# AzureLeon1/DiffSpectra

Hardware: AMD Instinct MI355X
Metric: molecules/sec, 1000-step QM9S all-spectra sampling (partial run) (higher is better)
Workload: dtype f32 (GEMMs as split-fp16 x3 MFMA with fp32 accumulate; fp32-level accuracy, parity gates unchanged)

## Files before the change

__graft_entry__.py:

```python
from __future__ import annotations

import os
import subprocess
import sys

ROOT = os.path.dirname(os.path.abspath(__file__))
if ROOT not in sys.path:
    sys.path.insert(0, ROOT)

CSRC = os.path.join(ROOT, "diffspectra_amd", "csrc")
HIP_SOURCES = [os.path.join(CSRC, n) for n in ("ds_forward.hip", "ds_gemm.hip", "ds_sampler.hip", "ds_spec.hip", "ds_aux.hip", "ds_match.hip", "ds_graph.hip", "ds_mces.hip", "ds_morgan.hip", "ds_subgeom.hip", "ds_mmd.hip", "ds_sets.hip", "ds_valence.hip", "ds_groups.hip", "ds_scaffold.hip", "ds_smiles.hip", "ds_substructure.hip", "ds_stereo.hip", "ds_brics.hip", "ds_mobile.hip", "ds_key.hip", "ds_fraggle.hip", "ds_bestrmsd.hip", "ds_reader.hip", "ds_train.hip", "ds_train_gemm.hip", "ds_train_attn.hip", "ds_train_chain.hip")]
HIP_DEPS = [os.path.join(CSRC, "ds_device.h"), os.path.join(CSRC, "ds_host.h"), os.path.join(CSRC, "ds_train_common.h"), os.path.join(CSRC, "ds_svd3.h"), os.path.join(CSRC, "ds_records.h"), os.path.join(CSRC, "ds_bonds.h"), os.path.join(CSRC, "ds_refine.h"), os.path.join(CSRC, "ds_perceive.h"), os.path.join(CSRC, "ds_mobile.h"), os.path.join(CSRC, "ds_vec.h"), os.path.join(CSRC, "ds_sites.h"),
            os.path.join(ROOT, "include", "diffspectra_hip.h"), os.path.join(ROOT, "include", "diffspectra_train.h"),
            os.path.join(ROOT, "include", "diffspectra_sets.h"), os.path.join(ROOT, "include", "diffspectra_valence.h"), os.path.join(ROOT, "include", "diffspectra_groups.h"),
            os.path.join(ROOT, "include", "diffspectra_scaffold.h"), os.path.join(ROOT, "include", "diffspectra_smiles.h"), os.path.join(ROOT, "include", "diffspectra_substructure.h"), os.path.join(ROOT, "include", "diffspectra_stereo.h"), os.path.join(ROOT, "include", "diffspectra_brics.h"), os.path.join(ROOT, "include", "diffspectra_mobile.h"), os.path.join(ROOT, "include", "diffspectra_key.h"), os.path.join(ROOT, "include", "diffspectra_fraggle.h"), os.path.join(ROOT, "include", "diffspectra_rmsd.h"), os.path.join(ROOT, "include", "diffspectra_reader.h"),
            os.path.join(ROOT, "include", "diffspectra_tiles.h"), os.path.join(ROOT, "include", "diffspectra_step.h"), os.path.join(ROOT, "include", "diffspectra_solver.h")]
LIB = os.path.join(ROOT, "diffspectra_amd", "libdiffspectra_hip.so")
OBJ_DIR = os.path.join(ROOT, "build", "obj")
BASE_FLAGS = ["--offload-arch=gfx950", "-O3", "-std=c++17", "-fPIC", "-Wno-pass-failed", "-Wno-unused-value"]
OPT_FLAGS = ["-mllvm", "-amdgpu-mfma-vgpr-form=1"]
LIBRARY_STATE = "not built"


def _digest(paths):
    import hashlib
    h = hashlib.sha1()
    for p in paths:
        h.update(os.path.basename(p).encode() + b"\0")
        with open(p, "rb") as f:
            h.update(f.read())
    return h.hexdigest()


def _read(path):
    try:
        with open(path) as f:
            return f.read()
    except OSError:
        return None


def _stale(target, deps):
    return not os.path.exists(target) or any(not os.path.exists(d) for d in deps) or _read(target + ".src") != _digest(deps)


def _compile(hipcc, src, obj, flags):
    cmd = [hipcc, *flags, "-c", src, "-o", obj]
    print("[build]", " ".join(cmd), file=sys.stderr, flush=True)
    r = subprocess.run(cmd, cwd=ROOT, capture_output=True, text=True)
# ... 83 lines not shown
```

diffspectra_amd/abi.py:

```python
from __future__ import annotations

import ctypes as C
import os
import re
import struct as _struct
from typing import Dict, List, NamedTuple, Tuple

_INCLUDE = os.path.join(os.path.dirname(os.path.dirname(os.path.abspath(__file__))), "include")

_FIELD_CODES = {"int64_t": "q", "int32_t": "i", "uint32_t": "I", "uint64_t": "Q", "float": "f"}
_CTYPES = {"P": C.c_void_p, "q": C.c_int64, "i": C.c_int32, "I": C.c_uint32, "Q": C.c_uint64, "f": C.c_float}
_ARG_CTYPES = {"*": C.c_void_p, "int": C.c_int, "int32_t": C.c_int32, "int64_t": C.c_int64, "uint32_t": C.c_uint32, "uint64_t": C.c_uint64,
               "float": C.c_float, "double": C.c_double}


class Prototype(NamedTuple):
    name: str
    ret: str
    params: List[Tuple[str, str]]

    @property
    def argtypes(self):
        return [_ARG_CTYPES[t] for _, t in self.params]

# ... 65 lines not shown
        return [name for name in self.prototypes if name.startswith(prefix)]

    def bind(self, lib: C.CDLL) -> None:
        for p in self.prototypes.values():
            fn = getattr(lib, p.name)
            fn.restype = None if p.ret == "void" else C.c_int
            fn.argtypes = p.argtypes

    def packer(self, name: str) -> _struct.Struct:
        return _struct.Struct("@" + "".join(code for _, code in self.structs[name]))

    def ctypes_struct(self, name: str):
        def ctype(code):
            return _CTYPES[code[-1]] * int(code[:-1]) if len(code) > 1 else _CTYPES[code]
        return type(name, (C.Structure,), {"_fields_": [(f_, ctype(code)) for f_, code in self.structs[name]]})


SAMPLING = Header("diffspectra_hip.h")
TRAINING = Header("diffspectra_train.h")
SETS = Header("diffspectra_sets.h")
VALENCE = Header("diffspectra_valence.h")
GROUPS = Header("diffspectra_groups.h")
SCAFFOLD = Header("diffspectra_scaffold.h")
SMILES = Header("diffspectra_smiles.h")
SUBSTRUCTURE = Header("diffspectra_substructure.h")
STEREO = Header("diffspectra_stereo.h")
BRICS = Header("diffspectra_brics.h")
MOBILE = Header("diffspectra_mobile.h")
KEY = Header("diffspectra_key.h")
FRAGGLE = Header("diffspectra_fraggle.h")
RMSD = Header("diffspectra_rmsd.h")
READER = Header("diffspectra_reader.h")
TILES = Header("diffspectra_tiles.h")
STEP = Header("diffspectra_step.h")
SOLVER = Header("diffspectra_solver.h")
```

diffspectra_amd/csrc/ds_forward.hip:

```cpp
#include <hip/hip_runtime.h>
#include <math.h>
#include <stdint.h>
#include <stdlib.h>

#include <atomic>
#include <mutex>
#include <utility>
#include <vector>

#include "../../include/diffspectra_hip.h"
#include "../../include/diffspectra_step.h"
#include "../../include/diffspectra_tiles.h"
#include "ds_device.h"
#include "ds_host.h"

#define ADAC DS_ADA_COLS
constexpr int DS_NODE_PF = 8;
constexpr int DS_NODE_PF2 = 4;
constexpr int DS_QKV_PF = 4;
constexpr int DS_QKV_PF_WIDE = 4;
constexpr int DS_NODE_TILE64_MIN_PER_CU = 4;
constexpr int DS_TWO_STREAM_MAX_PAIRS = 400000;

#ifdef DS_STAMPS
#define DS_STAMP_INIT()                                                                                 \
  unsigned long long _sa[16] = {0, 0, 0, 0, 0, 0, 0, 0, 0, 0, 0, 0, 0, 0, 0, 0};                        \
  unsigned long long _t0 = __builtin_amdgcn_s_memtime()
#define DS_STAMP(i)                                                                                     \
  do {                                                                                                  \
    const unsigned long long _t1 = __builtin_amdgcn_s_memtime();                                        \
    _sa[i] += _t1 - _t0;                                                                                \
    _t0 = _t1;                                                                                          \
  } while (0)
#define DS_STAMP_W(i)                                                                                   \
  do {                                                                                                  \
    asm volatile("s_waitcnt vmcnt(0) lgkmcnt(0)" ::: "memory");                                         \
    DS_STAMP(i);                                                                                        \
  } while (0)
#define DS_STAMP_FLUSH(t)                                                                               \
  do {                                                                                                  \
    if (threadIdx.x == (t))                                                                             \
      for (int _i = 0; _i < 16; ++_i)                                                                   \
        if (_sa[_i]) atomicAdd(reinterpret_cast<unsigned long long*>(c.ws.flags + 16) + _i, _sa[_i]);   \
  } while (0)
#else
#define DS_STAMP_INIT()
#define DS_STAMP(i)
#define DS_STAMP_W(i)
#define DS_STAMP_FLUSH(t)
#endif

namespace {

using dst::clear;
using dst::record;
using dst::wait;

struct Ctx {
  ds_layout L;
  ds_workspace ws;
  const float* wbase;
  const int64_t* woff;
  float edge_th, cutoff;
};

__device__ __forceinline__ const float* BW(const Ctx& c, int blk, int slot) {
  return c.wbase + c.woff[blk * DS_W_BLOCK_SLOTS + slot];
}
__device__ __forceinline__ const float* GW(const Ctx& c, int slot) {
  return c.wbase + c.woff[DS_NBLOCKS * DS_W_BLOCK_SLOTS + slot];
}

__device__ __forceinline__ float rbf_feature(float x, int k, const float* __restrict__ mean, const float* __restrict__ stdv,
                                             const float* __restrict__ astd) {
  if (k == 0) return x;
  const float z = (x - mean[k - 1]) / stdv[k - 1];
  return expf(-0.5f * (z * z)) / astd[k - 1];
}

__global__ void k_time_feat(Ctx c, const float* __restrict__ noise_level, int rows) {
  const int b = blockIdx.x * blockDim.x + threadIdx.x;
  if (b >= rows) return;
  const float* w = GW(c, DS_GW_SIN_W);
  const float x = noise_level[b];
  float* f = c.ws.tfeat + (size_t)b * 24;
  f[0] = x;
  for (int i = 0; i < 8; ++i) {
    const float fr = ((x * w[i]) * 2.0f) * 3.14159265358979323846f;
    f[1 + i] = sinf(fr);
    f[9 + i] = cosf(fr);
  }
  for (int i = 17; i < 24; ++i) f[i] = 0.0f;
}

__global__ void k_pair_flags(Ctx c, const float* __restrict__ cond_x, const float* __restrict__ cond_edge_x) {
  const int p = blockIdx.x * blockDim.x + threadIdx.x;
// ... 245 lines not shown
        }
      }
#pragma unroll
      for (int ps = 0; ps < 2; ++ps) {
        const int row = RW * wv + 8 * half + 4 * ps + g;
        ln_mod_quad256(v[ps], sh[ps], sc[ps]);
#pragma unroll
        for (int u = 0; u < 4; ++u)
          split_store4(&Xh[row][0], 256, 64 * u + 4 * j, row0 + row < c.L.Nn ? v[ps][u] : make_float4(0, 0, 0, 0));
      }
    }
  }
  __syncthreads();
  const float* bias = BW(c, blk, DS_BW_QKV_B) + col0;
  float* qkv = c.ws.qkv + (size_t)row0 * 768 + col0;
  const int valid = c.L.Nn - row0, wave = tid >> 6;
  for (int ch = wave; ch < NCH; ch += NW) {
    asm volatile("" ::: "memory");
    const float b = bias[ch * 32 + (tid & 31)];
    f32x16 acc[2], lo[2];
#pragma unroll
    for (int m = 0; m < 2; ++m)
#pragma unroll
      for (int i = 0; i < 16; ++i) acc[m][i] = b;
    acc_zero<2>(lo);
    wave_mma_h_ring<2, false, 16, PF>(&Xh[0][0], 256, BW(c, blk, DS_BW_QKV_H), 768, 256, col0 + ch * 32, 0, acc, lo);
    split_finish<2>(acc, lo);
    acc_store<2, 768>(acc, qkv + ch * 32, valid, [](int, float v) { return v; });
  }
}
__global__ __launch_bounds__(256) void k_node_qkv(Ctx c, int blk) { node_qkv_tile<4, DS_QKV_PF>(c, blk); }
__global__ __launch_bounds__(512, 2) void k_node_qkv_wide(Ctx c, int blk) { node_qkv_tile<8, DS_QKV_PF_WIDE>(c, blk); }

__global__ __launch_bounds__(1024) void k_attn_fused(Ctx c, int blk) {
  ds_fp16_saturate();
  DS_STAMP_INIT();
  constexpr int NT = 1024, QS = 512 + 32, LDT = 256 + 4, LDY = 2 * 64 + 8, CR = 32, MAXP = DS_MAX_ATOMS * (DS_MAX_ATOMS - 1) / 2;
  __shared__ __attribute__((aligned(16))) float QK[DS_MAX_ATOMS * QS];
  __shared__ __attribute__((aligned(16))) float Tt[2][CR][LDT];
  __shared__ __attribute__((aligned(16))) _Float16 Yc[2][CR][LDY];
  __shared__ __attribute__((aligned(16))) float AL[2][CR][32];
  __shared__ int PT[(MAXP + 15) & ~15];
  __shared__ int VT[32][32];
  static_assert(DS_MAX_ATOMS <= 32 && MAXP <= 511 - CR, "visit table packing");
  static_assert(DS_MAX_ATOMS * 128 <= 4 * NT && DS_MAX_ATOMS * 64 <= 2 * NT && MAXP <= NT, "single-pass staging");
  const int tid = threadIdx.x, wave = tid >> 6, lane = tid & 63, hh = lane >> 5;
  int n0, n, p0, P;
  if (c.L.mol_by_size) {
    const int4 r = reinterpret_cast<const int4*>(c.L.mol_by_size)[blockIdx.x];
    n0 = r.x; n = r.y; p0 = r.z; P = r.w;
  } else {
    const int m = blockIdx.x;
    n0 = c.L.node_off[m]; n = c.L.node_off[m + 1] - n0;
    p0 = c.L.pair_off[m]; P = c.L.pair_off[m + 1] - p0;
  }
  const WStreamH ws_e0 = wstream_h(BW(c, blk, DS_BW_E0_H), 256, 64, (wave & 7) * 32);
  const WStreamH ws_e1 = wstream_h(BW(c, blk, DS_BW_E1_H), 256, 64, (wave & 7) * 32);
  if (n <= 0) return;
  if (P <= 0) {
    for (int i = tid; i < 256; i += NT) c.ws.attn[(size_t)n0 * 256 + i] = 0.0f;
    return;
  }
  const int nch = (P + CR - 1) / CR;
  const bool producer = wave >= 8;
  const int ptid = tid & 511, prow = ptid >> 4, ppiece = ptid & 15;
  const u32x4* ye4 = reinterpret_cast<const u32x4*>(c.ws.ye) + (size_t)p0 * 16;
  auto row_pair = [&](int R) {
    const int d = R / n + 1, i = R - (d - 1) * n;
    int j = i + d;
    if (j >= n) j -= n;
    const int a = min(i, j), b = max(i, j);
    return a * (2 * n - a - 1) / 2 + (b - a - 1);
  };
  auto fetch_y = [&](int ck, bool class_order) {
    const int R = ck * CR + prow;
    const int Rc = min(R, P - 1);
    return ye4[(size_t)(class_order ? PT[Rc] : Rc) * 16 + ppiece];
  };
  auto commit_y = [&](int buf, const u32x4& v) { *reinterpret_cast<u32x4*>(&Yc[buf][prow][ppiece * 8]) = v; };
  h8 wf[2][4];
  auto load_weights = [&](const WStreamH& ws_) {
#pragma unroll
    for (int pl = 0; pl < 2; ++pl)
#pragma unroll
      for (int kb = 0; kb < 4; ++kb) wf[pl][kb] = wload_h(ws_, pl, kb);
  };
  auto project = [&](int buf) {
    f32x16 acc[1], lo[1];
    acc_zero<1>(acc);
    acc_zero<1>(lo);
// ... 50 lines not shown
    }
    f32x4 v[4];
#pragma unroll
    for (int u = 0; u < 4; ++u) {
      const int idx = min(tid + u * NT, n * 128 - 1);
      v[u] = reinterpret_cast<const f32x4*>(c.ws.qkv + (size_t)(n0 + (idx >> 7)) * 768)[idx & 127];
    }
    __builtin_amdgcn_sched_barrier(0);
    auto store_qk = [&]() {
      f32x4* junk = reinterpret_cast<f32x4*>(&Tt[1][0][0]) + tid;
#pragma unroll
      for (int u = 0; u < 4; ++u) {
        const int idx = tid + u * NT;
        f32x4* dst = idx < n * 128 ? reinterpret_cast<f32x4*>(QK) + (idx >> 7) * (QS / 4) + (idx & 127) : junk;
        *dst = v[u];
      }
    };
    if (producer) commit_y(0, y0);
    __syncthreads();
    if (producer) { DS_STAMP(8); } else { DS_STAMP(0); }
    if (producer) {
      produce(y1, y2, false, store_qk);
      load_weights(ws_e1);
    } else {
      store_qk();
      __syncthreads();
      DS_STAMP(1);
      const int row = tid >> 4, hs = tid & 15;
      for (int k = 0; k < nch; ++k) {
        const int pl = k * CR + row;
        if (pl < P) {
          const int e_ = PT[pl];
          float* out = c.ws.lg + (size_t)(p0 + pl) * 32;
          if (hs == 14) {
            const float h0 = (e_ & 0x10000) ? 1.0f : -1e10f, h1 = (e_ & 0x20000) ? 1.0f : -1e10f;
            out[0] = h0; out[1] = h1; out[16] = h0; out[17] = h1;
          } else if (hs < 14) {
            const int a = (e_ >> 8) & 255, b = e_ & 255;
            typedef const volatile f32x2 __attribute__((address_space(3))) * lds_v2;
            lds_v2 t0 = (lds_v2)(&Tt[k & 1][row][hs * 18]);
            lds_v2 qa = (lds_v2)(QK + a * QS + hs * 18);
            lds_v2 qb = (lds_v2)(QK + b * QS + hs * 18);
            lds_v2 ka = (lds_v2)(QK + a * QS + 256 + hs * 18);
            lds_v2 kb = (lds_v2)(QK + b * QS + 256 + hs * 18);
            float s_ab = 0.0f, s_ba = 0.0f;
#pragma unroll
            for (int j0 = 0; j0 < 9; j0 += 3) {
              f32x2 e[3], xa[3], xb[3], ya[3], yb[3];
#pragma unroll
              for (int j = 0; j < 3; ++j) { e[j] = t0[j0 + j]; xa[j] = qa[j0 + j]; xb[j] = qb[j0 + j]; ya[j] = ka[j0 + j]; yb[j] = kb[j0 + j]; }
#pragma unroll
              for (int j = 0; j < 3; ++j) {
                s_ab = __builtin_fmaf(xb[j].x * ya[j].x, e[j].x, s_ab); s_ab = __builtin_fmaf(xb[j].y * ya[j].y, e[j].y, s_ab);
                s_ba = __builtin_fmaf(xa[j].x * yb[j].x, e[j].x, s_ba); s_ba = __builtin_fmaf(xa[j].y * yb[j].y, e[j].y, s_ba);
              }
            }
            out[2 + hs] = s_ab / 4.0f;
            out[16 + 2 + hs] = s_ba / 4.0f;
          }
        }
        DS_STAMP(2);
        __syncthreads();
        DS_STAMP(3);
      }
    }
  }
  __threadfence_block();
  __syncthreads();
  float* V = QK;
  int* ET = reinterpret_cast<int*>(&Tt[0][0][0]);
  {
    const int t = tid >> 5, q = tid & 31, d = (q >> 1) + 1;
    int e = 511;
    if (t < n && q < n - 1) {
      int i, s_;
      if (2 * d == n) {
        i = t < d ? t : t - d;
        s_ = t < d ? t + d : t - d;
      } else {
        int sa = t + d, ib = t - d;
        if (sa >= n) sa -= n;
        if (ib < 0) ib += n;
        const bool first_is_a = t < ib;
        const bool take_a = (q & 1) ? !first_is_a : first_is_a;
        i = take_a ? t : ib;
        s_ = take_a ? sa : ib;
      }
      e = ((d - 1) * n + i) | (s_ << 9) | ((s_ < t ? 0 : 1) << 14);
    }
    VT[t][q] = e;
    const int s = q;
    int eo = -1;
    if (t < n && s < n && s != t) {
      const int lo_ = s < t ? s : t, hi_ = s < t ? t : s;
      eo = (lo_ * (2 * n - lo_ - 1) / 2 + (hi_ - lo_ - 1)) * 32 + (s < t ? 0 : 16);
    }
    ET[t * 32 + s] = eo;
    if (tid < P) PT[tid] = row_pair(tid);
  }
  f32x4 vst[2];
#pragma unroll
  for (int u = 0; u < 2; ++u) {
    const int i0 = min(tid + u * NT, n * 64 - 1);
    vst[u] = reinterpret_cast<const f32x4*>(c.ws.qkv + (size_t)(n0 + (i0 >> 6)) * 768 + 512)[i0 & 63];
  }
  __builtin_amdgcn_sched_barrier(0);
  __syncthreads();
  u32x4 y0 = {0, 0, 0, 0}, y1 = y0, y2 = y0;
  if (producer) {
    y0 = fetch_y(0, true);
    y1 = fetch_y(1, true);
    y2 = fetch_y(2, true);
  }
  auto store_v = [&]() {
    f32x4* junk = reinterpret_cast<f32x4*>(&Yc[0][0][0]) + tid;
#pragma unroll
    for (int u = 0; u < 2; ++u) {
      f32x4* dst = tid + u * NT < n * 64 ? reinterpret_cast<f32x4*>(V) + tid + u * NT : junk;
      *dst = vst[u];
    }
  };
  {
    const int h = lane & 15, sq = (lane >> 4) & 1, t = 2 * wave + hh;
    const int* et = ET + t * 32 + sq;
    float* lgm = c.ws.lg + (size_t)p0 * 32 + h;
    if (t < n) {
      float x[15];
      int eos[15];
      float mx = -INFINITY;
#pragma unroll
      for (int j = 0; j < 15; ++j) eos[j] = et[2 * j];
#pragma unroll
      for (int j = 0; j < 15; ++j) x[j] = lgm[max(eos[j], 0)];
      __builtin_amdgcn_sched_barrier(0);
#pragma unroll
      for (int j = 0; j < 15; ++j) x[j] = eos[j] >= 0 ? x[j] : -INFINITY;
#pragma unroll
      for (int j = 0; j < 15; ++j) mx = fmaxf(mx, x[j]);
      mx = fmaxf(mx, __shfl_xor(mx, 16, 64));
      float sum = 0.0f;
#pragma unroll
      for (int j = 0; j < 15; ++j) {
        x[j] = __expf(x[j] - mx);
        sum += x[j];
      }
      sum += __shfl_xor(sum, 16, 64);
      const float den = sum + 1e-16f;
#pragma unroll
      for (int j = 0; j < 15; ++j)
        if (eos[j] >= 0) lgm[eos[j]] = x[j] / den;
    }
  }
  store_v();
  __threadfence_block();
  __syncthreads();
  if (producer) { DS_STAMP(12); } else { DS_STAMP(4); }
  if (producer) {
    commit_y(0, y0);
    __syncthreads();
    produce(y1, y2, true, [] {});
    DS_STAMP_FLUSH(512);
  } else {
    const int arow = (tid & 255) >> 3, apiece = tid & 7;
    auto fetch_a = [&](int ck) {
      const int R = ck * CR + arow;
      return reinterpret_cast<const u32x4*>(c.ws.lg + (size_t)(p0 + PT[min(R, P - 1)]) * 32)[apiece];
    };
    auto commit_a = [&](int buf, const u32x4& v) {
      if (tid < 256) reinterpret_cast<u32x4*>(&AL[buf][arow][0])[apiece] = v;
    };
    const u32x4 a0 = fetch_a(0);
    u32x4 ab = fetch_a(1), aa = fetch_a(2);
    commit_a(0, a0);
    __syncthreads();
    __syncthreads();
    DS_STAMP(5);
    const int t_me = tid >> 4, q16 = tid & 15;
    const int* vt_row = &VT[t_me][0];
    int vt_q = 0, vt_e = vt_row[0];
    float4 acc[4];
#pragma unroll
    for (int u = 0; u < 4; ++u) acc[u] = make_float4(0, 0, 0, 0);
    auto interval = [&](int k, u32x4& A) {
      if (k + 1 < nch) commit_a((k + 1) & 1, A);
      if (k + 3 < nch) A = fetch_a(k + 3);
      const int R0 = k * CR;
      while ((vt_e & 511) - R0 < CR) {
        const int r = (vt_e & 511) - R0, s_ = (vt_e >> 9) & 31;
        const float4* gp = reinterpret_cast<const float4*>(&Tt[k & 1][r][4 * q16]);
        const float4* vp = reinterpret_cast<const float4*>(V + s_ * 256 + 4 * q16);
        const float* ap = &AL[k & 1][r][((vt_e >> 14) & 1) * 16 + (q16 >> 2)];
        float4 g[4], v[4];
        float al[4];
#pragma unroll
        for (int u = 0; u < 4; ++u) { g[u] = gp[16 * u]; v[u] = vp[16 * u]; al[u] = ap[4 * u]; }
        vt_e = vt_row[++vt_q];
#pragma unroll
        for (int u = 0; u < 4; ++u) {
          acc[u].x += (v[u].x * g[u].x) * al[u]; acc[u].y += (v[u].y * g[u].y) * al[u];
          acc[u].z += (v[u].z * g[u].z) * al[u]; acc[u].w += (v[u].w * g[u].w) * al[u];
        }
      }
      DS_STAMP(6);
      __syncthreads();
      DS_STAMP(7);
    };
    for (int k = 0; k < nch; k += 2) {
      interval(k, ab);
      if (k + 1 >= nch) break;
      interval(k + 1, aa);
    }
    if (t_me < n) {
      float4* o = reinterpret_cast<float4*>(c.ws.attn + (size_t)(n0 + t_me) * 256 + 4 * q16);
#pragma unroll
      for (int u = 0; u < 4; ++u) o[16 * u] = acc[u];
    }
    DS_STAMP_FLUSH(0);
  }
}

__global__ __launch_bounds__(256) void k_node_n2e(Ctx c, int blk) {
  ds_fp16_saturate();
  constexpr int T = 64, LDH = 2 * 256 + 8;
  __shared__ __attribute__((aligned(16))) _Float16 A1[T][LDH];
  const int tid = threadIdx.x, wave = tid >> 6, lane = tid & 63, row0 = blockIdx.x * T;
  const int Nn = c.L.Nn;
  {
    float4 v[16];
#pragma unroll
    for (int u = 0; u < 16; ++u) {
      const int idx = tid + u * 256, row = idx >> 6, k4 = idx & 63;
      v[u] = reinterpret_cast<const float4*>(c.ws.attn + (size_t)min(row0 + row, Nn - 1) * 256)[k4];
    }
#pragma unroll
    for (int u = 0; u < 16; ++u) {
      const int idx = tid + u * 256, row = idx >> 6, k4 = idx & 63;
      split_store4(&A1[row][0], 256, 4 * k4, row0 + row < Nn ? v[u] : make_float4(0, 0, 0, 0));
    }
  }
  __syncthreads();
  const int mt = wave >> 1, cc = wave & 1;
  if (row0 + mt * 32 >= Nn) return;
  f32x16 acc[1], lo[1];
  acc_zero<1>(acc);
// ... 1089 lines not shown
  const int m = blockIdx.x * blockDim.x + threadIdx.x;
  if (m >= c.L.B) return;
  const int n0 = c.L.node_off[m], n = c.L.node_off[m + 1] - n0;
  const bool nan = c.ws.flags[1] != 0;
  float sx = 0.0f, sy = 0.0f, sz = 0.0f;
  for (int a = 0; a < n; ++a) {
    const float* pp = c.ws.pos + (size_t)(n0 + a) * 4;
    if (!nan) { sx += pp[0]; sy += pp[1]; sz += pp[2]; }
  }
  const float fn = (float)n;
  for (int a = 0; a < n; ++a) {
    const float* pp = c.ws.pos + (size_t)(n0 + a) * 4;
    float* o = out_xh + (size_t)c.L.node_dense[n0 + a] * 9;
    const float px = nan ? 0.0f : pp[0], py = nan ? 0.0f : pp[1], pz = nan ? 0.0f : pp[2];
    o[0] = px - sx / fn; o[1] = py - sy / fn; o[2] = pz - sz / fn;
  }
}

__global__ void k_temb_finish(Ctx c, const float* __restrict__ tm3, int tm3_rows, const float* __restrict__ ctx) {
  ds_fp16_saturate();
  const size_t i = (size_t)blockIdx.x * blockDim.x + threadIdx.x;
  if (i >= (size_t)c.L.B * 1024) return;
  const size_t b = i >> 10, col = i & 1023;
  float v = tm3[(tm3_rows == 1 ? 0 : b) * 1024 + col];
  if (ctx) v += ctx[i];
  split_store1(reinterpret_cast<_Float16*>(c.ws.temb_silu) + b * 2048, 1024, (int)col, ds_silu(v));
}

bool make_ctx(Ctx& c, const ds_weights* w, const ds_layout* L, const ds_workspace* ws) {
  if (!w || !L || !ws || !w->base || !w->off_dev) return false;
  if (L->max_n > DS_MAX_ATOMS || L->B <= 0) return false;
  c.L = *L; c.ws = *ws; c.wbase = w->base; c.woff = w->off_dev;
  c.edge_th = w->edge_th; c.cutoff = w->spatial_cut_off;
  return true;
}

constexpr int MAX_DEVICES = 16;

inline int device_cus() {
  static std::atomic<int> cus[MAX_DEVICES];
  int dev = 0, n = 0;
  if (hipGetDevice(&dev) != hipSuccess || dev < 0 || dev >= MAX_DEVICES) return 256;
  if ((n = cus[dev].load(std::memory_order_relaxed)) > 0) return n;
  if (hipDeviceGetAttribute(&n, hipDeviceAttributeMultiprocessorCount, dev) != hipSuccess || n <= 0) n = 256;
  cus[dev].store(n, std::memory_order_relaxed);
  return n;
}

enum ProfSlot { PROF_EDGE_GEOM = 0, PROF_NODE_QKV = 1, PROF_ATTN = 2, PROF_NODE_UPDATE = 3, PROF_EDGE_UPDATE = 4, PROF_EQUI_PAIRS = 5 };
struct ProfState {
  int kernel = -1;
  int every = 1;
  long long seen = 0;
  std::vector<std::pair<hipEvent_t, hipEvent_t>> pool;
  size_t used = 0;
};
ProfState g_prof;

struct ProfScope {
  hipStream_t s;
  bool on = false;
  ProfScope(int kernel, hipStream_t st) : s(st) {
    if (g_prof.kernel != kernel) return;
    if ((g_prof.seen++ % g_prof.every) != 0 || g_prof.used >= g_prof.pool.size()) return;
    on = true;
    (void)hipEventRecord(g_prof.pool[g_prof.used].first, s);
  }
  ~ProfScope() {
    if (on) (void)hipEventRecord(g_prof.pool[g_prof.used++].second, s);
  }
};

void launch_edge_geom(const Ctx& c, int blk, hipStream_t s) {
  if (c.L.Pp <= 0) return;
  ProfScope ps(PROF_EDGE_GEOM, s);
  hipLaunchKernelGGL(k_edge_geom, dim3((c.L.Pp + 63) / 64), dim3(256), 0, s, c, blk);
}
int g_node_tile = -1;
bool node_tile64(const Ctx& c) {
  static const int env_tile = [] { const char* e = getenv("DIFFSPECTRA_NODE_TILE"); return e ? atoi(e) : -1; }();
  const int pick = g_node_tile > 0 ? g_node_tile : env_tile;
  if (pick == 32 || pick == 64) return pick == 64;
  return (c.L.Nn + 63) / 64 >= DS_NODE_TILE64_MIN_PER_CU * device_cus();
}
void launch_node_qkv(const Ctx& c, int blk, hipStream_t s) {
  ProfScope ps(PROF_NODE_QKV, s);
  if (node_tile64(c)) hipLaunchKernelGGL(k_node_qkv_wide, dim3((c.L.Nn + 63) / 64), dim3(512), 0, s, c, blk);
  else hipLaunchKernelGGL(k_node_qkv, dim3((c.L.Nn + 63) / 64, 2), dim3(256), 0, s, c, blk);
}
void launch_attn(const Ctx& c, int blk, hipStream_t s) {
  ProfScope ps(PROF_ATTN, s);
  hipLaunchKernelGGL(k_attn_fused, dim3(c.L.B), dim3(1024), 0, s, c, blk);
}
void launch_node_n2e(const Ctx& c, int blk, hipStream_t s) { hipLaunchKernelGGL(k_node_n2e, dim3((c.L.Nn + 63) / 64), dim3(256), 0, s, c, blk); }
template <bool N2E>
void launch_node_update(const Ctx& c, int blk, hipStream_t s) {
  ProfScope ps(PROF_NODE_UPDATE, s);
  if (node_tile64(c)) hipLaunchKernelGGL(k_node_update64<N2E>, dim3((c.L.Nn + 63) / 64), dim3(512), 0, s, c, blk);
  else hipLaunchKernelGGL(k_node_update<N2E>, dim3((c.L.Nn + 31) / 32), dim3(256), 0, s, c, blk);
}
void launch_edge_update(const Ctx& c, int blk, hipStream_t s) {
  if (c.L.Pp <= 0) return;
  ProfScope ps(PROF_EDGE_UPDATE, s);
  hipLaunchKernelGGL(k_edge_update, dim3((c.L.Pp + 127) / 128), dim3(256), 0, s, c, blk);
}
void launch_equi_pairs(const Ctx& c, int blk, hipStream_t s) {
  if (c.L.Pp <= 0) return;
  ProfScope ps(PROF_EQUI_PAIRS, s);
  hipLaunchKernelGGL(k_equi_pairs, dim3(min((c.L.Pp + 31) / 32, device_cus())), dim3((EQUI_NCW + EQUI_NLW) * 64), 0, s, c, blk);
}
void launch_pos_update(const Ctx& c, int last, hipStream_t s) { hipLaunchKernelGGL(k_pos_update, dim3(c.L.B), dim3(64), 0, s, c, last); }

}

extern "C" {

void ds_struct_sizes(int64_t* out) {
  out[0] = sizeof(ds_weights);
  out[1] = sizeof(ds_layout);
  out[2] = sizeof(ds_workspace);
  out[3] = sizeof(ds_gemm_args);
}

static int stage_time(const ds_weights* w, const ds_layout* L, ds_workspace* ws, const float* noise_level, const float* ctx_emb,
// ... 12 lines not shown
  float* tm3 = ws->ada;
  g.A = ws->tmid; g.lda = 1024; g.Wp = w->base + off[DS_GW_TM3_W]; g.bias = w->base + off[DS_GW_TM3_B];
  g.C = tm3; g.K = 1024; g.act = 0;
  st = dst::gemm_routed_as(&g, B, stream);
  if (st) return st;
  const size_t tot = (size_t)B * 1024;
  hipLaunchKernelGGL(k_temb_finish, dim3((unsigned)((tot + 255) / 256)), dim3(256), 0, s, c, (const float*)tm3, rows, ctx_emb);
  static_assert(ADAC % 32 == 0, "adaLN table width");
  return ds_gemm_split(ws->temb_silu, w->base + off[DS_GW_ADA_W], w->base + off[DS_GW_ADA_B], ws->ada, ADAC, B, 1024, ADAC, stream);
}

int ds_stage_time(const ds_weights* w, const ds_layout* L, ds_workspace* ws, const float* noise_level, const float* ctx_emb,
                  void* stream) {
  return L ? stage_time(w, L, ws, noise_level, ctx_emb, L->B, stream) : DS_ERR_ARG;
}

int ds_stage_time_uniform(const ds_weights* w, const ds_layout* L, ds_workspace* ws, const float* noise_level, const float* ctx_emb,
                          void* stream) {
  return stage_time(w, L, ws, noise_level, ctx_emb, 1, stream);
}

int ds_stage_init(const ds_weights* w, const ds_layout* L, ds_workspace* ws, const float* xh, const float* edge_x,
                  const float* cond_x, const float* cond_edge_x, void* stream) {
  hipStream_t s = (hipStream_t)stream;
  Ctx c;
  if (!make_ctx(c, w, L, ws) || !xh || !edge_x || ((cond_x == nullptr) != (cond_edge_x == nullptr))) return DS_ERR_ARG;
  if (!clear(ws->flags, 8 * sizeof(int32_t), s)) return DS_ERR_LAUNCH;
  if (L->Pp > 0) hipLaunchKernelGGL(k_pair_flags, dim3((L->Pp + 1023) / 1024), dim3(1024), 0, s, c, cond_x, cond_edge_x);
  hipLaunchKernelGGL(k_node_init, dim3((L->Nn + 7) / 8), dim3(256), 0, s, c, xh, cond_x);
  if (L->Pp > 0) hipLaunchKernelGGL(k_pair_init, dim3((L->Pp + 63) / 64), dim3(256), 0, s, c, edge_x, cond_x, cond_edge_x);
  return DST_CHECK_LAUNCH();
}

int ds_stage_block(const ds_weights* w, const ds_layout* L, ds_workspace* ws, int blk, int last, void* stream) {
  hipStream_t s = (hipStream_t)stream;
  Ctx c;
  if (!make_ctx(c, w, L, ws) || blk < 0 || blk >= DS_NBLOCKS) return DS_ERR_ARG;
  launch_edge_geom(c, blk, s);
  launch_node_qkv(c, blk, s);
  launch_attn(c, blk, s);
  launch_node_update<true>(c, blk, s);
  launch_edge_update(c, blk, s);
  launch_equi_pairs(c, blk, s);
  launch_pos_update(c, last, s);
  return DST_CHECK_LAUNCH();
}

int ds_stage_readout(const ds_weights* w, const ds_layout* L, ds_workspace* ws, float* out_xh, float* out_edge, void* stream) {
  hipStream_t s = (hipStream_t)stream;
  Ctx c;
  if (!make_ctx(c, w, L, ws) || !out_xh || !out_edge) return DS_ERR_ARG;
  const size_t nx = (size_t)L->B * L->N * 9, ne = (size_t)L->B * L->N * L->N * 2;
  if (!clear(out_xh, nx * sizeof(float), s) || !clear(out_edge, ne * sizeof(float), s)) return DS_ERR_LAUNCH;
  hipLaunchKernelGGL(k_node_readout, dim3((L->Nn + 31) / 32), dim3(256), 0, s, c, out_xh);
  if (L->Pp > 0) hipLaunchKernelGGL(k_edge_readout, dim3((L->Pp + 127) / 128), dim3(256), 0, s, c, out_edge);
  hipLaunchKernelGGL(k_final_pos, dim3((L->B + 63) / 64), dim3(64), 0, s, c, out_xh);
  return DST_CHECK_LAUNCH();
}

struct SideStream {
  hipStream_t s = nullptr;
  hipEvent_t fork[DS_NBLOCKS + 1] = {}, join[DS_NBLOCKS + 1] = {};
  std::once_flag once;
  bool ok = false;
};
static SideStream g_side[MAX_DEVICES];
static int g_two_stream = -1;

static SideStream* side_stream() {
  int dev = 0;
  if (hipGetDevice(&dev) != hipSuccess || dev < 0 || dev >= MAX_DEVICES) return nullptr;
  SideStream& ss = g_side[dev];
  std::call_once(ss.once, [&ss] {
    bool ok = hipStreamCreateWithFlags(&ss.s, hipStreamNonBlocking) == hipSuccess;
    for (int i = 0; ok && i <= DS_NBLOCKS; ++i)
      ok = hipEventCreateWithFlags(&ss.fork[i], hipEventDisableTiming) == hipSuccess &&
           hipEventCreateWithFlags(&ss.join[i], hipEventDisableTiming) == hipSuccess;
    ss.ok = ok;
  });
  return ss.ok ? &ss : nullptr;
}

static int forward_blocks_two_streams(const ds_weights* w, const ds_layout* L, ds_workspace* ws, hipStream_t s, SideStream* ss) {
  Ctx c;
  if (!make_ctx(c, w, L, ws)) return DS_ERR_ARG;
  hipStream_t s2 = ss->s;
  const hipEvent_t fork0 = ss->fork[DS_NBLOCKS], join0 = ss->join[DS_NBLOCKS];
  if (!record(fork0, s) || !wait(s2, fork0)) return DS_ERR_LAUNCH;
  launch_node_qkv(c, 0, s2);
  if (!record(join0, s2)) return DS_ERR_LAUNCH;
  for (int blk = 0; blk < DS_NBLOCKS; ++blk) {
    launch_edge_geom(c, blk, s);
    if (!wait(s, blk == 0 ? join0 : ss->join[blk - 1])) return DS_ERR_LAUNCH;
    launch_attn(c, blk, s);
    launch_node_n2e(c, blk, s);
    if (!record(ss->fork[blk], s) || !wait(s2, ss->fork[blk])) return DS_ERR_LAUNCH;
    launch_node_update<false>(c, blk, s2);
    if (blk + 1 < DS_NBLOCKS) launch_node_qkv(c, blk + 1, s2);
    if (!record(ss->join[blk], s2)) return DS_ERR_LAUNCH;
    launch_edge_update(c, blk, s);
    if (!wait(s, ss->join[blk])) return DS_ERR_LAUNCH;
    launch_equi_pairs(c, blk, s);
    launch_pos_update(c, blk == DS_NBLOCKS - 1 ? 1 : 0, s);
  }
  return DST_CHECK_LAUNCH();
}

int ds_set_two_stream(int on) {
  const int prev = g_two_stream;
  g_two_stream = on;
  return prev;
}

int ds_set_node_tile(int rows) {
  const int prev = g_node_tile;
  g_node_tile = (rows == 32 || rows == 64) ? rows : -1;
  return prev;
}

static int forward(const ds_weights* w, const ds_layout* L, ds_workspace* ws, const float* xh, const float* edge_x, const float* cond_x,
                   const float* cond_edge_x, const float* noise_level, const float* ctx_emb, float* out_xh, float* out_edge,
                   bool uniform, void* stream) {
  int st = uniform ? ds_stage_time_uniform(w, L, ws, noise_level, ctx_emb, stream) : ds_stage_time(w, L, ws, noise_level, ctx_emb, stream);
  if (st) return st;
  st = ds_stage_init(w, L, ws, xh, edge_x, cond_x, cond_edge_x, stream);
  if (st) return st;
  static const int env_two = [] { const char* e = getenv("DIFFSPECTRA_TWO_STREAM"); return e ? atoi(e) : -1; }();
  const int pick = g_two_stream >= 0 ? g_two_stream : env_two;
  const int two = pick >= 0 ? pick : (L->Pp < DS_TWO_STREAM_MAX_PAIRS ? 1 : 0);
  SideStream* ss = two ? side_stream() : nullptr;
  if (ss) {
    st = forward_blocks_two_streams(w, L, ws, (hipStream_t)stream, ss);
    if (st) return st;
  } else {
    for (int b = 0; b < DS_NBLOCKS; ++b) {
      st = ds_stage_block(w, L, ws, b, b == DS_NBLOCKS - 1, stream);
      if (st) return st;
    }
  }
  return ds_stage_readout(w, L, ws, out_xh, out_edge, stream);
}

int ds_forward(const ds_weights* w, const ds_layout* L, ds_workspace* ws, const float* xh, const float* edge_x,
               const float* cond_x, const float* cond_edge_x, const float* noise_level, const float* ctx_emb, float* out_xh,
               float* out_edge, void* stream) {
  return forward(w, L, ws, xh, edge_x, cond_x, cond_edge_x, noise_level, ctx_emb, out_xh, out_edge, false, stream);
}

int ds_forward_uniform(const ds_weights* w, const ds_layout* L, ds_workspace* ws, const float* xh, const float* edge_x,
                       const float* cond_x, const float* cond_edge_x, const float* noise_level, const float* ctx_emb, float* out_xh,
                       float* out_edge, void* stream) {
  return forward(w, L, ws, xh, edge_x, cond_x, cond_edge_x, noise_level, ctx_emb, out_xh, out_edge, true, stream);
}

int ds_profile_config(int kernel, int every, int max_samples) {
  for (auto& e : g_prof.pool) { (void)hipEventDestroy(e.first); (void)hipEventDestroy(e.second); }
  g_prof.pool.clear();
  g_prof.used = 0; g_prof.seen = 0;
  g_prof.kernel = kernel; g_prof.every = every > 0 ? every : 1;
  if (kernel < 0) return DS_OK;
  if (kernel > 6 || max_samples <= 0) return DS_ERR_ARG;
  g_prof.pool.resize((size_t)max_samples);
  for (auto& e : g_prof.pool)
    if (hipEventCreate(&e.first) != hipSuccess || hipEventCreate(&e.second) != hipSuccess) return DS_ERR_LAUNCH;
  return DS_OK;
}

int ds_profile_read(double* total_ms, int64_t* samples) {
  if (!total_ms || !samples) return DS_ERR_ARG;
// ... 14 lines not shown
```

diffspectra_amd/engine.py:

```python
from __future__ import annotations

import ctypes as C
import os
from typing import Dict, List, Optional

import numpy as np
import torch

from . import abi
from .abi import ptr

_ptr = ptr

LIB_PATH = os.environ.get("DIFFSPECTRA_HIP_LIB", os.path.join(os.path.dirname(os.path.abspath(__file__)), "libdiffspectra_hip.so"))

_HDR = abi.SAMPLING
HEADER_PATH = _HDR.path
CONSTS = _HDR.consts
BLOCK_SLOTS, GLOBAL_SLOTS = _HDR.enums["ds_block_slot"], _HDR.enums["ds_global_slot"]
EXPORTS = _HDR.exports("ds_")
NB = CONSTS["DS_NBLOCKS"]
W_BLOCK_SLOTS, W_GLOBAL_SLOTS, W_NUM_SLOTS = CONSTS["DS_W_BLOCK_SLOTS"], CONSTS["DS_W_GLOBAL_SLOTS"], CONSTS["DS_W_NUM_SLOTS"]
ADA_COLS = CONSTS["DS_ADA_COLS"]
ADA_STRIDE = CONSTS["DS_ADA_BLOCK_STRIDE"]
# ... 2 lines not shown
DsWeights = _HDR.ctypes_struct("ds_weights")
DsLayout = _HDR.ctypes_struct("ds_layout")
DsWorkspace = _HDR.ctypes_struct("ds_workspace")
DsGemmArgs = _HDR.ctypes_struct("ds_gemm_args")
_WS_FIELDS = [f for f, _ in _HDR.structs["ds_workspace"]]

_lib = None


def load_library() -> C.CDLL:
    global _lib
    if _lib is not None:
        return _lib
    if not os.path.exists(LIB_PATH):
        raise RuntimeError(f"{LIB_PATH} is missing: build it with `python -c 'import __graft_entry__ as g; g.build()'`. "
                           "diffspectra_amd has no CPU/PyTorch fallback.")
    lib = C.CDLL(LIB_PATH)
    abi.SAMPLING.bind(lib)
    abi.TRAINING.bind(lib)
    abi.SETS.bind(lib)
    abi.VALENCE.bind(lib)
    abi.GROUPS.bind(lib)
    abi.SCAFFOLD.bind(lib)
    abi.SMILES.bind(lib)
    abi.SUBSTRUCTURE.bind(lib)
    abi.STEREO.bind(lib)
    abi.BRICS.bind(lib)
    abi.MOBILE.bind(lib)
    abi.KEY.bind(lib)
    abi.FRAGGLE.bind(lib)
    abi.RMSD.bind(lib)
    abi.READER.bind(lib)
    abi.TILES.bind(lib)
    abi.STEP.bind(lib)
    abi.SOLVER.bind(lib)
    sizes = (C.c_int64 * 4)()
    lib.ds_struct_sizes(sizes)
    mine = [C.sizeof(t) for t in (DsWeights, DsLayout, DsWorkspace, DsGemmArgs)]
    if list(sizes) != mine:
        raise RuntimeError(f"C-ABI struct layout mismatch: library {list(sizes)} vs binding {mine}")
    _lib = lib
    return lib


def _check(status: int, what: str):
    if status != 0:
        raise RuntimeError(f"{what} failed with status {status} "
                           f"({ {-1: 'bad argument', -2: 'HIP launch error'}.get(status, 'unknown')})")


def _stream():
    return torch.cuda.current_stream().cuda_stream


def _f32c(t: torch.Tensor, device) -> torch.Tensor:
    return t.detach().to(device=device, dtype=torch.float32).contiguous()



def pack_linear(weight: torch.Tensor, n_pad_to: int = 32) -> torch.Tensor:
    w = weight.detach().to(torch.float32).cpu()
    N, K = w.shape
    Kp, Np = (K + 7) // 8 * 8, (N + n_pad_to - 1) // n_pad_to * n_pad_to
    b = torch.zeros(Kp, Np)
    b[:K, :N] = w.t()
    return b.view(Kp // 8, 2, 4, Np).permute(0, 1, 3, 2).contiguous().reshape(-1)
# ... 1113 lines not shown
```

Before: 245.4.

## Keep attention logits resident in LDS instead of round-tripping through global memory

When the pair logits for a molecule fit in the unused tail of the QK shared buffer plus the AL staging buffer, the fused attention kernel writes logits, runs the softmax and reads the attention weights directly from LDS, with the address packed into the per-edge VT entry. This removes the global-memory write/read of ws.lg, the block fences, and the AL prefetch pipeline in the aggregation loop. The path is on by default in the full forward and two-stream paths, can be toggled by env var or API, and is off when a staged caller may observe lg. The packed LDS address limits the bits available in the VT encoding.

```diff
diff --git a/__graft_entry__.py b/__graft_entry__.py
--- a/__graft_entry__.py
+++ b/__graft_entry__.py
@@ -14,7 +14,7 @@
             os.path.join(ROOT, "include", "diffspectra_hip.h"), os.path.join(ROOT, "include", "diffspectra_train.h"),
             os.path.join(ROOT, "include", "diffspectra_sets.h"), os.path.join(ROOT, "include", "diffspectra_valence.h"), os.path.join(ROOT, "include", "diffspectra_groups.h"),
             os.path.join(ROOT, "include", "diffspectra_scaffold.h"), os.path.join(ROOT, "include", "diffspectra_smiles.h"), os.path.join(ROOT, "include", "diffspectra_substructure.h"), os.path.join(ROOT, "include", "diffspectra_stereo.h"), os.path.join(ROOT, "include", "diffspectra_brics.h"), os.path.join(ROOT, "include", "diffspectra_mobile.h"), os.path.join(ROOT, "include", "diffspectra_key.h"), os.path.join(ROOT, "include", "diffspectra_fraggle.h"), os.path.join(ROOT, "include", "diffspectra_rmsd.h"), os.path.join(ROOT, "include", "diffspectra_reader.h"),
-            os.path.join(ROOT, "include", "diffspectra_tiles.h"), os.path.join(ROOT, "include", "diffspectra_step.h"), os.path.join(ROOT, "include", "diffspectra_solver.h")]
+            os.path.join(ROOT, "include", "diffspectra_tiles.h"), os.path.join(ROOT, "include", "diffspectra_attn.h"), os.path.join(ROOT, "include", "diffspectra_step.h"), os.path.join(ROOT, "include", "diffspectra_solver.h")]
 LIB = os.path.join(ROOT, "diffspectra_amd", "libdiffspectra_hip.so")
 OBJ_DIR = os.path.join(ROOT, "build", "obj")
 BASE_FLAGS = ["--offload-arch=gfx950", "-O3", "-std=c++17", "-fPIC", "-Wno-pass-failed", "-Wno-unused-value"]
diff --git a/diffspectra_amd/abi.py b/diffspectra_amd/abi.py
--- a/diffspectra_amd/abi.py
+++ b/diffspectra_amd/abi.py
@@ -121,5 +121,6 @@
 RMSD = Header("diffspectra_rmsd.h")
 READER = Header("diffspectra_reader.h")
 TILES = Header("diffspectra_tiles.h")
+ATTN = Header("diffspectra_attn.h")
 STEP = Header("diffspectra_step.h")
 SOLVER = Header("diffspectra_solver.h")
diff --git a/diffspectra_amd/csrc/ds_forward.hip b/diffspectra_amd/csrc/ds_forward.hip
--- a/diffspectra_amd/csrc/ds_forward.hip
+++ b/diffspectra_amd/csrc/ds_forward.hip
@@ -5,9 +5,11 @@
 
 #include <atomic>
 #include <mutex>
+#include <type_traits>
 #include <utility>
 #include <vector>
 
+#include "../../include/diffspectra_attn.h"
 #include "../../include/diffspectra_hip.h"
 #include "../../include/diffspectra_step.h"
 #include "../../include/diffspectra_tiles.h"
@@ -62,6 +64,7 @@
   const float* wbase;
   const int64_t* woff;
   float edge_th, cutoff;
+  int attn_resident;
 };
 
 __device__ __forceinline__ const float* BW(const Ctx& c, int blk, int slot) {
@@ -373,10 +376,19 @@
 __global__ __launch_bounds__(256) void k_node_qkv(Ctx c, int blk) { node_qkv_tile<4, DS_QKV_PF>(c, blk); }
 __global__ __launch_bounds__(512, 2) void k_node_qkv_wide(Ctx c, int blk) { node_qkv_tile<8, DS_QKV_PF_WIDE>(c, blk); }
 
+constexpr int ATTN_QS = 512 + 32;
+constexpr int ATTN_CR = 32;
+static_assert(ATTN_QS % 32 == 0 && (ATTN_QS * 4) % 16 == 0, "the tail of QK behind n atoms starts 16-byte aligned and holds whole 32-float logit rows");
+typedef float __attribute__((address_space(3))) * lds_f32;
+__device__ __forceinline__ lds_f32 attn_lg_at(lds_f32 qk, lds_f32 al, int n, int off) {
+  const int tail = (DS_MAX_ATOMS - n) * ATTN_QS;
+  return off < tail ? qk + n * ATTN_QS + off : al + (off - tail);
+}
+__device__ __forceinline__ lds_f32 attn_lg_row(lds_f32 qk, lds_f32 al, int n, int p) { return attn_lg_at(qk, al, n, 32 * p); }
 __global__ __launch_bounds__(1024) void k_attn_fused(Ctx c, int blk) {
   ds_fp16_saturate();
   DS_STAMP_INIT();
-  constexpr int NT = 1024, QS = 512 + 32, LDT = 256 + 4, LDY = 2 * 64 + 8, CR = 32, MAXP = DS_MAX_ATOMS * (DS_MAX_ATOMS - 1) / 2;
+  constexpr int NT = 1024, QS = ATTN_QS, LDT = 256 + 4, LDY = 2 * 64 + 8, CR = ATTN_CR, MAXP = DS_MAX_ATOMS * (DS_MAX_ATOMS - 1) / 2;
   __shared__ __attribute__((aligned(16))) float QK[DS_MAX_ATOMS * QS];
   __shared__ __attribute__((aligned(16))) float Tt[2][CR][LDT];
   __shared__ __attribute__((aligned(16))) _Float16 Yc[2][CR][LDY];
@@ -387,6 +399,8 @@
   static_assert(DS_MAX_ATOMS * 128 <= 4 * NT && DS_MAX_ATOMS * 64 <= 2 * NT && MAXP <= NT, "single-pass staging");
   const int tid = threadIdx.x, wave = tid >> 6, lane = tid & 63, hh = lane >> 5;
   int n0, n, p0, P;
+  const float* w_e0 = BW(c, blk, DS_BW_E0_H);
+  const float* w_e1 = BW(c, blk, DS_BW_E1_H);
   if (c.L.mol_by_size) {
     const int4 r = reinterpret_cast<const int4*>(c.L.mol_by_size)[blockIdx.x];
     n0 = r.x; n = r.y; p0 = r.z; P = r.w;
@@ -395,8 +409,11 @@
     n0 = c.L.node_off[m]; n = c.L.node_off[m + 1] - n0;
     p0 = c.L.pair_off[m]; P = c.L.pair_off[m + 1] - p0;
   }
-  const WStreamH ws_e0 = wstream_h(BW(c, blk, DS_BW_E0_H), 256, 64, (wave & 7) * 32);
-  const WStreamH ws_e1 = wstream_h(BW(c, blk, DS_BW_E1_H), 256, 64, (wave & 7) * 32);
+  static_assert(sizeof(AL) % 128 == 0, "AL holds whole logit rows");
+  const bool resident = c.attn_resident != 0 && P * 128 <= (DS_MAX_ATOMS - n) * QS * 4 + (int)sizeof(AL);
+  const lds_f32 QKl = (lds_f32)QK, ALl = (lds_f32)&AL[0][0][0];
+  const WStreamH ws_e0 = wstream_h(w_e0, 256, 64, (wave & 7) * 32);
+  const WStreamH ws_e1 = wstream_h(w_e1, 256, 64, (wave & 7) * 32);
   if (n <= 0) return;
   if (P <= 0) {
     for (int i = tid; i < 256; i += NT) c.ws.attn[(size_t)n0 * 256 + i] = 0.0f;
@@ -513,9 +530,11 @@
         if (pl < P) {
           const int e_ = PT[pl];
           float* out = c.ws.lg + (size_t)(p0 + pl) * 32;
+          const lds_f32 outl = attn_lg_row(QKl, ALl, n, pl);
           if (hs == 14) {
             const float h0 = (e_ & 0x10000) ? 1.0f : -1e10f, h1 = (e_ & 0x20000) ? 1.0f : -1e10f;
-            out[0] = h0; out[1] = h1; out[16] = h0; out[17] = h1;
+            if (resident) { outl[0] = h0; outl[1] = h1; outl[16] = h0; outl[17] = h1; }
+            else { out[0] = h0; out[1] = h1; out[16] = h0; out[17] = h1; }
           } else if (hs < 14) {
             const int a = (e_ >> 8) & 255, b = e_ & 255;
             typedef const volatile f32x2 __attribute__((address_space(3))) * lds_v2;
@@ -536,8 +555,9 @@
                 s_ba = __builtin_fmaf(xa[j].x * yb[j].x, e[j].x, s_ba); s_ba = __builtin_fmaf(xa[j].y * yb[j].y, e[j].y, s_ba);
               }
             }
-            out[2 + hs] = s_ab / 4.0f;
-            out[16 + 2 + hs] = s_ba / 4.0f;
+            const float l_ab = s_ab / 4.0f, l_ba = s_ba / 4.0f;
+            if (resident) { outl[2 + hs] = l_ab; outl[16 + 2 + hs] = l_ba; }
+            else { out[2 + hs] = l_ab; out[16 + 2 + hs] = l_ba; }
           }
         }
         DS_STAMP(2);
@@ -546,7 +566,7 @@
       }
     }
   }
-  __threadfence_block();
+  if (!resident) __threadfence_block();
   __syncthreads();
   float* V = QK;
   int* ET = reinterpret_cast<int*>(&Tt[0][0][0]);
@@ -568,6 +588,11 @@
         s_ = take_a ? sa : ib;
       }
       e = ((d - 1) * n + i) | (s_ << 9) | ((s_ < t ? 0 : 1) << 14);
+      if (resident) {
+        const int lo_ = s_ < t ? s_ : t, hi_ = s_ < t ? t : s_;
+        const lds_f32 ar = attn_lg_row(QKl, ALl, n, lo_ * (2 * n - lo_ - 1) / 2 + (hi_ - lo_ - 1)) + (s_ < t ? 0 : 16);
+        e |= (int)(((unsigned)(size_t)ar >> 4) << 15);
+      }
     }
     VT[t][q] = e;
     const int s = q;
@@ -611,8 +636,14 @@
       float mx = -INFINITY;
 #pragma unroll
       for (int j = 0; j < 15; ++j) eos[j] = et[2 * j];
-#pragma unroll
-      for (int j = 0; j < 15; ++j) x[j] = lgm[max(eos[j], 0)];
+      auto lg_at = [&](int eo) { return attn_lg_at(QKl, ALl, n, eo) + h; };
+      if (resident) {
+#pragma unroll
+        for (int j = 0; j < 15; ++j) x[j] = *lg_at(max(eos[j], 0));
+      } else {
+#pragma unroll
+        for (int j = 0; j < 15; ++j) x[j] = lgm[max(eos[j], 0)];
+      }
       __builtin_amdgcn_sched_barrier(0);
 #pragma unroll
       for (int j = 0; j < 15; ++j) x[j] = eos[j] >= 0 ? x[j] : -INFINITY;
@@ -627,13 +658,19 @@
       }
       sum += __shfl_xor(sum, 16, 64);
       const float den = sum + 1e-16f;
-#pragma unroll
-      for (int j = 0; j < 15; ++j)
-        if (eos[j] >= 0) lgm[eos[j]] = x[j] / den;
+      if (resident) {
+#pragma unroll
+        for (int j = 0; j < 15; ++j)
+          if (eos[j] >= 0) *lg_at(eos[j]) = x[j] / den;
+      } else {
+#pragma unroll
+        for (int j = 0; j < 15; ++j)
+          if (eos[j] >= 0) lgm[eos[j]] = x[j] / den;
+      }
     }
   }
   store_v();
-  __threadfence_block();
+  if (!resident) __threadfence_block();
   __syncthreads();
   if (producer) { DS_STAMP(12); } else { DS_STAMP(4); }
   if (producer) {
@@ -650,47 +687,57 @@
     auto commit_a = [&](int buf, const u32x4& v) {
       if (tid < 256) reinterpret_cast<u32x4*>(&AL[buf][arow][0])[apiece] = v;
     };
-    const u32x4 a0 = fetch_a(0);
-    u32x4 ab = fetch_a(1), aa = fetch_a(2);
-    commit_a(0, a0);
-    __syncthreads();
-    __syncthreads();
-    DS_STAMP(5);
     const int t_me = tid >> 4, q16 = tid & 15;
-    const int* vt_row = &VT[t_me][0];
-    int vt_q = 0, vt_e = vt_row[0];
     float4 acc[4];
 #pragma unroll
     for (int u = 0; u < 4; ++u) acc[u] = make_float4(0, 0, 0, 0);
-    auto interval = [&](int k, u32x4& A) {
-      if (k + 1 < nch) commit_a((k + 1) & 1, A);
-      if (k + 3 < nch) A = fetch_a(k + 3);
-      const int R0 = k * CR;
-      while ((vt_e & 511) - R0 < CR) {
-        const int r = (vt_e & 511) - R0, s_ = (vt_e >> 9) & 31;
-        const float4* gp = reinterpret_cast<const float4*>(&Tt[k & 1][r][4 * q16]);
-        const float4* vp = reinterpret_cast<const float4*>(V + s_ * 256 + 4 * q16);
-        const float* ap = &AL[k & 1][r][((vt_e >> 14) & 1) * 16 + (q16 >> 2)];
-        float4 g[4], v[4];
-        float al[4];
-#pragma unroll
-        for (int u = 0; u < 4; ++u) { g[u] = gp[16 * u]; v[u] = vp[16 * u]; al[u] = ap[4 * u]; }
-        vt_e = vt_row[++vt_q];
-#pragma unroll
-        for (int u = 0; u < 4; ++u) {
-          acc[u].x += (v[u].x * g[u].x) * al[u]; acc[u].y += (v[u].y * g[u].y) * al[u];
-          acc[u].z += (v[u].z * g[u].z) * al[u]; acc[u].w += (v[u].w * g[u].w) * al[u];
+    auto aggregate = [&](auto res_flag) {
+      constexpr bool RES = decltype(res_flag)::value;
+      u32x4 ab = {0, 0, 0, 0}, aa = ab;
+      if constexpr (!RES) {
+        const u32x4 a0 = fetch_a(0);
+        ab = fetch_a(1); aa = fetch_a(2);
+        commit_a(0, a0);
+      }
+      __syncthreads();
+      __syncthreads();
+      DS_STAMP(5);
+      const int* vt_row = &VT[t_me][0];
+      int vt_q = 0, vt_e = vt_row[0];
+      auto interval = [&](int k, u32x4& A) {
+        if constexpr (!RES) {
+          if (k + 1 < nch) commit_a((k + 1) & 1, A);
+          if (k + 3 < nch) A = fetch_a(k + 3);
         }
-      }
-      DS_STAMP(6);
-      __syncthreads();
-      DS_STAMP(7);
+        const int R0 = k * CR;
+        while ((vt_e & 511) - R0 < CR) {
+          const int r = (vt_e & 511) - R0, s_ = (vt_e >> 9) & 31;
+          const float4* gp = reinterpret_cast<const float4*>(&Tt[k & 1][r][4 * q16]);
+          const float4* vp = reinterpret_cast<const float4*>(V + s_ * 256 + 4 * q16);
+          const lds_f32 ap = (RES ? (lds_f32)(size_t)(((unsigned)vt_e >> 15) << 4) : (lds_f32)&AL[k & 1][r][((vt_e >> 14) & 1) * 16]) + (q16 >> 2);
+          float4 g[4], v[4];
+          float al[4];
+#pragma unroll
+          for (int u = 0; u < 4; ++u) { g[u] = gp[16 * u]; v[u] = vp[16 * u]; al[u] = ap[4 * u]; }
+          vt_e = vt_row[++vt_q];
+#pragma unroll
+          for (int u = 0; u < 4; ++u) {
+            acc[u].x += (v[u].x * g[u].x) * al[u]; acc[u].y += (v[u].y * g[u].y) * al[u];
+            acc[u].z += (v[u].z * g[u].z) * al[u]; acc[u].w += (v[u].w * g[u].w) * al[u];
+          }
+        }
+        DS_STAMP(6);
+        __syncthreads();
+        DS_STAMP(7);
+      };
+      for (int k = 0; k < nch; k += 2) {
+        interval(k, ab);
+        if (k + 1 >= nch) break;
+        interval(k + 1, aa);
+      }
     };
-    for (int k = 0; k < nch; k += 2) {
-      interval(k, ab);
-      if (k + 1 >= nch) break;
-      interval(k + 1, aa);
-    }
+    if (resident) aggregate(std::true_type{});
+    else aggregate(std::false_type{});
     if (t_me < n) {
       float4* o = reinterpret_cast<float4*>(c.ws.attn + (size_t)(n0 + t_me) * 256 + 4 * q16);
 #pragma unroll
@@ -1846,6 +1893,7 @@
   if (L->max_n > DS_MAX_ATOMS || L->B <= 0) return false;
   c.L = *L; c.ws = *ws; c.wbase = w->base; c.woff = w->off_dev;
   c.edge_th = w->edge_th; c.cutoff = w->spatial_cut_off;
+  c.attn_resident = 0;
   return true;
 }
 
@@ -1902,8 +1950,15 @@
   if (node_tile64(c)) hipLaunchKernelGGL(k_node_qkv_wide, dim3((c.L.Nn + 63) / 64), dim3(512), 0, s, c, blk);
   else hipLaunchKernelGGL(k_node_qkv, dim3((c.L.Nn + 63) / 64, 2), dim3(256), 0, s, c, blk);
 }
-void launch_attn(const Ctx& c, int blk, hipStream_t s) {
+int g_attn_resident = -1;
+bool attn_resident(bool lg_observed) {
+  static const int env_res = [] { const char* e = getenv("DIFFSPECTRA_ATTN_RESIDENT"); return e ? atoi(e) : -1; }();
+  const int pick = g_attn_resident >= 0 ? g_attn_resident : env_res;
+  return pick >= 0 ? pick != 0 : !lg_observed;
+}
+void launch_attn(Ctx c, int blk, hipStream_t s, bool lg_observed) {
   ProfScope ps(PROF_ATTN, s);
+  c.attn_resident = attn_resident(lg_observed) ? 1 : 0;
   hipLaunchKernelGGL(k_attn_fused, dim3(c.L.B), dim3(1024), 0, s, c, blk);
 }
 void launch_node_n2e(const Ctx& c, int blk, hipStream_t s) { hipLaunchKernelGGL(k_node_n2e, dim3((c.L.Nn + 63) / 64), dim3(256), 0, s, c, blk); }
@@ -1982,18 +2037,22 @@
   return DST_CHECK_LAUNCH();
 }
 
-int ds_stage_block(const ds_weights* w, const ds_layout* L, ds_workspace* ws, int blk, int last, void* stream) {
+static int stage_block(const ds_weights* w, const ds_layout* L, ds_workspace* ws, int blk, int last, bool lg_observed, void* stream) {
   hipStream_t s = (hipStream_t)stream;
   Ctx c;
   if (!make_ctx(c, w, L, ws) || blk < 0 || blk >= DS_NBLOCKS) return DS_ERR_ARG;
   launch_edge_geom(c, blk, s);
   launch_node_qkv(c, blk, s);
-  launch_attn(c, blk, s);
+  launch_attn(c, blk, s, lg_observed);
   launch_node_update<true>(c, blk, s);
   launch_edge_update(c, blk, s);
   launch_equi_pairs(c, blk, s);
   launch_pos_update(c, last, s);
   return DST_CHECK_LAUNCH();
+}
+
+int ds_stage_block(const ds_weights* w, const ds_layout* L, ds_workspace* ws, int blk, int last, void* stream) {
+  return stage_block(w, L, ws, blk, last, true, stream);
 }
 
 int ds_stage_readout(const ds_weights* w, const ds_layout* L, ds_workspace* ws, float* out_xh, float* out_edge, void* stream) {
@@ -2042,7 +2101,7 @@
   for (int blk = 0; blk < DS_NBLOCKS; ++blk) {
     launch_edge_geom(c, blk, s);
     if (!wait(s, blk == 0 ? join0 : ss->join[blk - 1])) return DS_ERR_LAUNCH;
-    launch_attn(c, blk, s);
+    launch_attn(c, blk, s, false);
     launch_node_n2e(c, blk, s);
     if (!record(ss->fork[blk], s) || !wait(s2, ss->fork[blk])) return DS_ERR_LAUNCH;
     launch_node_update<false>(c, blk, s2);
@@ -2065,6 +2124,12 @@
 int ds_set_node_tile(int rows) {
   const int prev = g_node_tile;
   g_node_tile = (rows == 32 || rows == 64) ? rows : -1;
+  return prev;
+}
+
+int ds_set_attn_resident(int on) {
+  const int prev = g_attn_resident;
+  g_attn_resident = (on == 0 || on == 1) ? on : -1;
   return prev;
 }
 
@@ -2084,7 +2149,7 @@
     if (st) return st;
   } else {
     for (int b = 0; b < DS_NBLOCKS; ++b) {
-      st = ds_stage_block(w, L, ws, b, b == DS_NBLOCKS - 1, stream);
+      st = stage_block(w, L, ws, b, b == DS_NBLOCKS - 1, false, stream);
       if (st) return st;
     }
   }
diff --git a/diffspectra_amd/engine.py b/diffspectra_amd/engine.py
--- a/diffspectra_amd/engine.py
+++ b/diffspectra_amd/engine.py
@@ -58,6 +58,7 @@
     abi.RMSD.bind(lib)
     abi.READER.bind(lib)
     abi.TILES.bind(lib)
+    abi.ATTN.bind(lib)
     abi.STEP.bind(lib)
     abi.SOLVER.bind(lib)
     sizes = (C.c_int64 * 4)()
diff --git a/include/diffspectra_attn.h b/include/diffspectra_attn.h
--- /dev/null
+++ b/include/diffspectra_attn.h
@@ -0,0 +1,13 @@
+#ifndef DIFFSPECTRA_ATTN_H
+#define DIFFSPECTRA_ATTN_H
+
+#ifdef __cplusplus
+extern "C" {
+#endif
+
+int ds_set_attn_resident(int on);
+
+#ifdef __cplusplus
+}
+#endif
+#endif
```

New measurement: 245.0. No clear change (-0.2%).
